# stephane-caron/pink

Hardware: AMD Instinct MI355X
Metric: ik_qp_solves_per_s (higher is better)
Workload: dtype f64

## Files before the change

### emu/wave_emu.h

```cpp
#pragma once

#include <ucontext.h>

#include <cmath>
#include <cstdio>
#include <cstdlib>
#include <cstring>

#define __device__
#define __host__
#define __global__ inline
#define __forceinline__ inline
#define __launch_bounds__(x)
#define PINKHIP_OCCUPANCY_ATTR(NV)
#define PINKHIP_OCCUPANCY_PACKED(NV, DENSE)
#define PINKHIP_OCCUPANCY_SWEEP(NT)
#define PINKHIP_OCCUPANCY_SWEEP3(NV, MD, W)
#define PINKHIP_OCCUPANCY_SWEEPX(NV, MD)
#define PINKHIP_OCCUPANCY_ROLLOUT(NV)
#define PINKHIP_OCCUPANCY_FK
#define PINKHIP_OCCUPANCY_SMALL_STACK

#include "../pink_amd/csrc/fast_sincos.h"

struct EmuDim3 {
  unsigned x = 0, y = 0, z = 0;
};
static EmuDim3 blockIdx, threadIdx;

inline unsigned long long atomicMin(unsigned long long *p, unsigned long long v) {
  const unsigned long long old = *p;
  if (v < old) *p = v;
  return old;
}

namespace pinkhip {

constexpr int kWave = 64;

struct Emu {
  int cur = 0;
  long long block = 0;
  ucontext_t main_ctx;
  ucontext_t ctx[kWave];
  bool done[kWave];
  int live = 0;
  double slot_d[kWave];
  int slot_i[kWave];
  long long arrivals[kWave];
  int tag[kWave];
  alignas(16) double lds[20480];
  char *stacks = nullptr;
};

inline Emu &emu() {
  static Emu e;
  return e;
}

inline int lane_id() { return emu().cur; }
inline long long block_id() { return emu().block; }
inline double *shared_base() { return emu().lds; }

inline void emu_rendezvous(int tag) {
  Emu &e = emu();
  const int me = e.cur;
  e.arrivals[me]++;
  e.tag[me] = tag;
  int nxt = me;
  do {
    nxt = (nxt + 1) % kWave;
  } while (e.done[nxt] && nxt != me);
  if (nxt != me) {
    e.cur = nxt;
    swapcontext(&e.ctx[me], &e.ctx[nxt]);
  }
  for (int l = 0; l < kWave; ++l) {
    if (e.done[l]) continue;
    if (e.arrivals[l] != e.arrivals[me] && e.arrivals[l] != e.arrivals[me] + 1 &&
        e.arrivals[l] + 1 != e.arrivals[me]) {
      std::fprintf(stderr, "wave emulator: divergence at lane %d vs %d (tag %d vs %d)\n", me, l,
                   e.tag[me], e.tag[l]);
      std::abort();
    }
    if (e.arrivals[l] == e.arrivals[me] && e.tag[l] != e.tag[me]) {
      std::fprintf(stderr, "wave emulator: lanes %d and %d at different primitives (%d vs %d)\n", me,
                   l, e.tag[me], e.tag[l]);
      std::abort();
    }
  }
}

inline void wave_sync() { emu_rendezvous(1); }
inline void sched_fence() {}
inline void pin16(const double (&)[8], const double (&)[8]) {}
inline void pin8(const double (&)[4], const double (&)[4]) {}
template <typename T>
inline void pin(T &) {}
inline void opaque(double &) {}
inline int opaque_uniform(int x) { return x; }
template <class Args>
inline const Args *kernarg_reload(const Args &a) {
  return &a;
}

inline double bcast(double v, int src) {
  Emu &e = emu();
  e.slot_d[e.cur] = v;
  emu_rendezvous(2);
  if (src < 0 || src >= kWave) {
    std::fprintf(stderr, "wave emulator: bcast from lane %d\n", src);
    std::abort();
  }
  const double r = e.slot_d[src];
  emu_rendezvous(3);
  return r;
}

inline int bcast_i(int v, int src) {
  Emu &e = emu();
  e.slot_i[e.cur] = v;
  emu_rendezvous(4);
  if (src < 0 || src >= kWave) std::abort();
  const int r = e.slot_i[src];
  emu_rendezvous(5);
  return r;
}

inline double emu_exchange(double v, int partner_of_me, int tag) {
  Emu &e = emu();
  e.slot_d[e.cur] = v;
  emu_rendezvous(tag);
  const double o = e.slot_d[partner_of_me];
  emu_rendezvous(tag + 1);
  return o;
}

template <class Op>
inline double emu_reduce(double v, double ident, Op op, int tag) {
  const int l = emu().cur;
  v = op(v, emu_exchange(v, l ^ 1, tag));
  v = op(v, emu_exchange(v, l ^ 2, tag));
  v = op(v, emu_exchange(v, (l & ~7) | (7 - (l & 7)), tag));
  v = op(v, emu_exchange(v, (l & ~15) | (15 - (l & 15)), tag));
  const int row = l >> 4;
  double t = emu_exchange(v, (row == 1 || row == 3) ? (row - 1) * 16 + 15 : l, tag);
  v = op(v, (row == 1 || row == 3) ? t : ident);
  t = emu_exchange(v, 31, tag);
  v = op(v, (row >= 2) ? t : ident);
  return bcast(v, 63);
}
inline double wave_sum(double v) {
  return emu_reduce(v, 0.0, [](double a, double b) { return a + b; }, 6);
}
inline double wave_min(double v) {
  return emu_reduce(v, INFINITY, [](double a, double b) { return std::fmin(a, b); }, 8);
}

inline double key_pack(double v, int payload) {
  long long b;
  std::memcpy(&b, &v, 8);
  b = (b & ~0xFFLL) | (long long)(payload & 0xFF);
  std::memcpy(&v, &b, 8);
  return v;
}
inline int key_payload(double k) {
  long long b;
  std::memcpy(&b, &k, 8);
  return (int)(b & 0xFF);
}
inline double fast_rcp(double x) { return 1.0 / x; }
inline double fast_rsqrt(double x) { return 1.0 / std::sqrt(x); }
inline double fast_rcp1(double x) { return 1.0 / x; }
inline double max_raw(double a, double b) { return a > b ? a : b; }
inline double min_raw(double a, double b) { return a < b ? a : b; }
inline int wave_uniform(int v) { return v; }
inline double approx_rcp(double x) { return 1.0 / x; }
inline float approx_rcpf(float x) { return 1.0f / x; }
inline double fast_rsqrt1(double x) { return 1.0 / std::sqrt(x); }

inline bool wave_any(bool p) {
  Emu &e = emu();
  e.slot_i[e.cur] = p ? 1 : 0;
  emu_rendezvous(14);
  bool r = false;
  for (int l = 0; l < kWave; ++l) r = r || e.slot_i[l];
  emu_rendezvous(15);
  return r;
}
inline bool lanes_on(bool) { return true; }
inline unsigned long long wave_ballot(bool p) {
  Emu &e = emu();
  e.slot_i[e.cur] = p ? 1 : 0;
  emu_rendezvous(42);
  unsigned long long r = 0;
  for (int l = 0; l < kWave; ++l)
    if (e.slot_i[l]) r |= 1ull << l;
  emu_rendezvous(43);
  return r;
}
inline bool lane_pred(unsigned long long mask) { return ((mask >> emu().cur) & 1ull) != 0; }
template <int W>
constexpr unsigned long long mask_lane(int J) {
  unsigned long long m = 0;
  for (int g = 0; g < 64 / W; ++g) m |= 1ull << (g * W + J);
  return m;
}
template <int W>
constexpr unsigned long long mask_lanes_below(int J) {
  const unsigned long long low = (J >= 64) ? ~0ull : ((1ull << J) - 1ull);
  unsigned long long m = 0;
  for (int g = 0; g < 64 / W; ++g) m |= low << (g * W);
  return m;
}
template <int W>
constexpr unsigned long long mask_groups(unsigned bits) {
  constexpr unsigned long long all = (W >= 64) ? ~0ull : ((1ull << (W & 63)) - 1ull);
  unsigned long long m = 0;
  for (int g = 0; g < 64 / W; ++g) m |= ((bits >> g) & 1u) ? (all << (g * W)) : 0ull;
  return m;
}
template <int W>
constexpr unsigned long long mask_groups_of_lane(unsigned long long m, int K) {
  unsigned bits = 0;
  for (int g = 0; g < 64 / W; ++g) bits |= static_cast<unsigned>((m >> (g * W + K)) & 1ull) << g;
  return mask_groups<W>(bits);
}
template <int W>
inline int group_first_lane(bool p) {
  Emu &e = emu();
  e.slot_i[e.cur] = p ? 1 : 0;
  emu_rendezvous(40);
  int r = W;
  const int base = e.cur & ~(W - 1);
  for (int l = W - 1; l >= 0; --l)
    if (e.slot_i[base + l]) r = l;
  emu_rendezvous(41);
  return r;
}
inline double lane_shfl(double v, int src_lane) {
  if (src_lane < 0 || src_lane >= kWave) {
    std::fprintf(stderr, "wave emulator: lane_shfl from lane %d\n", src_lane);
    std::abort();
  }
  return emu_exchange(v, src_lane, 16);
}
inline int lane_shfl_i(int v, int src_lane) {
  Emu &e = emu();
  if (src_lane < 0 || src_lane >= kWave) std::abort();
  e.slot_i[e.cur] = v;
  emu_rendezvous(18);
  const int r = e.slot_i[src_lane];
// ... 229 lines not shown
```

### pink_amd/csrc/ik_stack_rows.h

```cpp
#pragma once

#include "ik_common.h"

namespace pinkhip {

struct HbmTerms {
  static constexpr bool kOnTheFly = false;
  double lb = 0.0, ub = 0.0, x = 0.0;
  int status = 0;
  __device__ __forceinline__ void frame_rows(int, double (&)[6]) const {}
  __device__ __forceinline__ double error(int) const { return 0.0; }
  __device__ __forceinline__ double diag_error(int) const { return 0.0; }
  __device__ __forceinline__ double dense_col(int) const { return 0.0; }
  __device__ __forceinline__ double dense_h(int) const { return 0.0; }
};

struct NoMid {
  __device__ __forceinline__ void operator()() const {}
};
template <int NX>
struct StackFront {
  double m[NX > 0 ? NX : 1] = {};
  double hxx[NX > 0 ? NX * (NX + 1) / 2 : 1] = {};
  double cx[NX > 0 ? NX : 1] = {};
};
struct WaveSplit {
  long long first = 0;
  unsigned rel = 0;
};
#ifndef PINKHIP_WAVE_SPLIT
#define PINKHIP_WAVE_SPLIT(Src) (!Src::kOnTheFly)
#endif
template <int NV, int W, int RCMAX, class Src, int DEPTH = 1, int NX = 0, bool DIAG = false, int NM, class Mid = NoMid>
__device__ __forceinline__ void stack_rows_bcast(const KernelArgs &a, long long b, Src *terms, bool in, int li,
                                                 double (&M)[NM], double &ci, double &mu_l, Mid mid = Mid(), StackFront<NX> *front = nullptr,
                                                 double *hdiag = nullptr, WaveSplit ws = WaveSplit()) {
  static_assert(NX >= 0 && NX <= 2 && (NX == 0 || !Src::kOnTheFly), "at most two front columns, from HBM");
  static_assert(NM >= NV && W >= 16, "row-group kernels only");
  using BcT = Bcast<W>;
  const int nv = a.nv, Kd = a.Kd, K = a.K;
  constexpr bool SPLIT = DIAG && PINKHIP_WAVE_SPLIT(Src);
  const double *Jb = a.J + (SPLIT ? ws.first : b) * (long long)Kd * nv;
  const double *eb = a.e + (SPLIT ? ws.first : b) * (long long)K;
  const double *costb = a.cost_batched ? a.cost + (SPLIT ? ws.first : b) * (long long)K : a.cost;
  const unsigned voJ = SPLIT ? ws.rel * static_cast<unsigned>(Kd * nv) + li : 0u;
  const unsigned voE = SPLIT ? ws.rel * static_cast<unsigned>(K) + li : 0u;
  const unsigned voC = (SPLIT && a.cost_batched) ? voE : static_cast<unsigned>(li);
  constexpr int RC = Src::kOnTheFly ? 6 : (RCMAX < 8 ? RCMAX : 8);
  constexpr int NB = Src::kOnTheFly ? 2 : DEPTH + 1;
  static_assert(RC <= 16, "weight rows are broadcast from the first row of 16 lanes");
  struct Chunk {
    double r[RC];
    double pw, pe, pg, pl;
    double px[NX > 0 ? NX : 1];
  };
  Chunk buf[NB];
  auto request = [&](Chunk &dst, int r0) {
    const int rc = (Kd - r0 < RC) ? Kd - r0 : RC;
    if constexpr (Src::kOnTheFly) {
      double six[6];
      terms->frame_rows(r0 / 6, six);
#pragma unroll
      for (int kk = 0; kk < RC; ++kk) dst.r[kk] = (in && kk < rc) ? six[kk] : 0.0;
    } else {
#pragma unroll
      for (int kk = 0; kk < RC; ++kk) {
        if constexpr (SPLIT) dst.r[kk] = (in && kk < rc) ? (Jb + (long long)(r0 + kk) * nv)[voJ] : 0.0;
        else dst.r[kk] = (in && kk < rc) ? Jb[(long long)(r0 + kk) * nv + li] : 0.0;
      }
    }
    dst.pw = dst.pe = dst.pg = dst.pl = 0.0;
    if constexpr (NX > 0) {
#pragma unroll
      for (int x = 0; x < NX; ++x) {
        if constexpr (SPLIT) dst.px[x] = (li < rc) ? (Jb + ((long long)r0 * nv - NX + x))[voJ - li + static_cast<unsigned>(li * nv)] : 0.0;
        else dst.px[x] = (li < rc) ? Jb[(long long)(r0 + li) * nv - NX + x] : 0.0;
      }
    }
    if (li < rc) {
      const int k = r0 + li;
      if constexpr (SPLIT) {
        dst.pw = (costb + r0)[voC];
        if constexpr (Src::kOnTheFly) dst.pe = terms->error(k);
        else dst.pe = (eb + r0)[voE];
        dst.pg = (a.row_gain + r0)[static_cast<unsigned>(li)];
        dst.pl = (a.row_lm + r0)[static_cast<unsigned>(li)];
      } else {
        dst.pw = costb[k];
        if constexpr (Src::kOnTheFly) dst.pe = terms->error(k);
        else dst.pe = eb[k];
        dst.pg = a.row_gain[k];
        dst.pl = a.row_lm[k];
      }
    }
  };
  if (Kd > 0) {
#pragma unroll
    for (int d = 0; d < NB - 1; ++d)
      if (d * RC < Kd) request(buf[d], d * RC);
  }
  mid();
  for (int r0 = 0; r0 < Kd; r0 += RC) {
    const int rc = (Kd - r0 < RC) ? Kd - r0 : RC;
    if (r0 + (NB - 1) * RC < Kd) request(buf[NB - 1], r0 + (NB - 1) * RC);
    const Chunk &cur = buf[0];
    const double wa = (li < rc) ? cur.pw * cur.pw : 0.0;
    const double gw = (li < rc) ? cur.pg * wa * cur.pe : 0.0;
    if (li < rc) mu_l += cur.pl * (cur.pg * cur.pg) * wa * cur.pe * cur.pe;
    const BcT wab = bcast_prepare<W>(wa), gwb = bcast_prepare<W>(gw);
    BcT pxb[NX > 0 ? NX : 1];
    if constexpr (NX > 0) {
      front->hxx[0] = fma(wa * cur.px[0], cur.px[0], front->hxx[0]);
      front->cx[0] = fma(gw, cur.px[0], front->cx[0]);
      if constexpr (NX == 2) {
        front->hxx[1] = fma(wa * cur.px[0], cur.px[1], front->hxx[1]);
        front->hxx[2] = fma(wa * cur.px[1], cur.px[1], front->hxx[2]);
        front->cx[1] = fma(gw, cur.px[1], front->cx[1]);
      }
#pragma unroll
      for (int x = 0; x < NX; ++x) pxb[x] = bcast_prepare<W>(cur.px[x]);
    }
    static_for<0, RC>([&](auto Kc) {
      constexpr int kk = decltype(Kc)::value;
      if (kk < rc) {
        const double aa = fma_bcast<W, kk>(0.0, wab, cur.r[kk]);
        ci = fma_bcast<W, kk>(ci, gwb, cur.r[kk]);
        if constexpr (DIAG) *hdiag = fma(cur.r[kk], aa, *hdiag);
        const BcT rowb = bcast_prepare<W>(cur.r[kk]);
        static_for<0, NV>([&](auto Jc) {
          constexpr int j = decltype(Jc)::value;
          M[j] = fma_bcast<W, j>(M[j], rowb, aa);
        });
        if constexpr (NX > 0) {
#pragma unroll
          for (int x = 0; x < NX; ++x) front->m[x] = fma_bcast<W, kk>(front->m[x], pxb[x], aa);
        }
      }
    });
#pragma unroll
    for (int d = 0; d + 1 < NB; ++d) buf[d] = buf[d + 1];
  }
}

template <class Src>
__device__ __forceinline__ double stack_diag_tasks(const KernelArgs &a, long long b, Src *terms, int li, double &ci,
                                                   double &mu_l) {
  const double *eb = a.e + b * (long long)a.K;
  const double *costb = a.cost_batched ? a.cost + b * (long long)a.K : a.cost;
  double dadd = 0.0;
  for (int t = 0; t < a.n_dtasks; ++t) {
    const int off = li - a.dtask_col0[t];
    if (off >= 0 && off < a.dtask_k[t]) {
      const int r = a.dtask_row0[t] + off;
      const double w = costb[r], gn = a.row_gain[r], l = a.row_lm[r];
      double ev;
      if constexpr (Src::kOnTheFly) ev = terms->diag_error(r);
      else ev = eb[r];
      const double wa = w * w;
      dadd += wa;
      ci += gn * wa * ev;
      mu_l += l * (gn * gn) * wa * ev * ev;
    }
  }
  return dadd;
}

template <class Src>
__device__ __forceinline__ double stack_diag_tasks(const KernelArgs &a, WaveSplit ws, Src *terms, int li, double &ci,
                                                   double &mu_l) {
  const double *eb = a.e + ws.first * (long long)a.K;
  const double *costb = a.cost_batched ? a.cost + ws.first * (long long)a.K : a.cost;
  const unsigned vo = ws.rel * static_cast<unsigned>(a.K);
  const unsigned voc = a.cost_batched ? vo : 0u;
  double dadd = 0.0;
  for (int t = 0; t < a.n_dtasks; ++t) {
    const int off = li - a.dtask_col0[t];
    if (off >= 0 && off < a.dtask_k[t]) {
      const int r = a.dtask_row0[t] + off;
      const double w = costb[voc + static_cast<unsigned>(r)], gn = a.row_gain[r], l = a.row_lm[r];
      double ev;
      if constexpr (Src::kOnTheFly) ev = terms->diag_error(r);
      else ev = eb[vo + static_cast<unsigned>(r)];
      const double wa = w * w;
      dadd += wa;
      ci += gn * wa * ev;
      mu_l += l * (gn * gn) * wa * ev * ev;
    }
  }
  return dadd;
}

}
```

### pink_amd/csrc/ik_sweep.h

```cpp
#pragma once

#include "ik_common.h"
#include "ik_kernels_packed.h"
#include "ik_stack_rows.h"

#ifdef PINKHIP_SECTION_CLOCK
#ifndef PINKHIP_TICK
static __device__ unsigned long long pinkhip_clock[16];
#define PINKHIP_TICK(k)                                                        \
  do {                                                                         \
    if (clock_on) {                                                            \
      const unsigned long long now_ = __builtin_readcyclecounter();            \
      if (lane == 0) atomicAdd(&pinkhip_clock[k], now_ - clock_prev);          \
      clock_prev = __builtin_readcyclecounter();                               \
    }                                                                          \
  } while (0)
#endif
#else
#ifndef PINKHIP_TICK
#define PINKHIP_TICK(k)
#endif
#endif

#ifndef PINKHIP_SWEEP_COLUMN_CHAINS
#define PINKHIP_SWEEP_COLUMN_CHAINS(NT) 2
#endif

#ifndef PINKHIP_SWEEP_CERT_TOL
#define PINKHIP_SWEEP_CERT_TOL 1e-12
#endif
#ifndef PINKHIP_STACK_DEPTH
#define PINKHIP_STACK_DEPTH 1
#endif
#ifndef PINKHIP_STACK_DEPTH_WIDE
#define PINKHIP_STACK_DEPTH_WIDE 2
#endif
#ifndef PINKHIP_SWEEP_INDEXED_COLUMN
#define PINKHIP_SWEEP_INDEXED_COLUMN 1
#endif
#ifndef PINKHIP_SWEEP_ROUTE_COND
#define PINKHIP_SWEEP_ROUTE_COND 1e8
#endif
#ifndef PINKHIP_SWEEP_PPM
#define PINKHIP_SWEEP_PPM 1
#endif
#ifndef PINKHIP_SWEEP_PPM_CRASH
#define PINKHIP_SWEEP_PPM_CRASH 1
#endif
#ifndef PINKHIP_ROLLOUT_PPM_DENSE
#define PINKHIP_ROLLOUT_PPM_DENSE 0
#endif
#ifndef PINKHIP_ROLLOUT_PPM_VIRTUAL
#define PINKHIP_ROLLOUT_PPM_VIRTUAL 0
#endif
#ifndef PINKHIP_SWEEP_PPM_DENSE
#define PINKHIP_SWEEP_PPM_DENSE 1
#endif
#ifdef PINKHIP_SWEEP_DEBUG_WHY
#define PINKHIP_WHY(k) why = (k) + 10 * status_before
#else
#define PINKHIP_WHY(k)
#endif
#ifndef PINKHIP_SWEEP_PPM_MIN_CURV
#define PINKHIP_SWEEP_PPM_MIN_CURV 1e-5
#endif
#ifndef PINKHIP_SWEEP_PPM_MURTY_AFTER
#define PINKHIP_SWEEP_PPM_MURTY_AFTER(nv) (4 * (nv) + 20)
#endif

#ifndef PINKHIP_SWEEP_DIAG_REGISTER
#define PINKHIP_SWEEP_DIAG_REGISTER(Src) (!Src::kOnTheFly)
#endif
#ifndef PINKHIP_SWEEP_LATE_ADDRESSES
#define PINKHIP_SWEEP_LATE_ADDRESSES(Src) (!Src::kOnTheFly)
#endif
#ifndef PINKHIP_SWEEP_LANE_MASKS
#define PINKHIP_SWEEP_LANE_MASKS(Src) (!Src::kOnTheFly)
#endif
#ifndef PINKHIP_SWEEP_SPLIT_CLOSING
#define PINKHIP_SWEEP_SPLIT_CLOSING(Src) (!Src::kOnTheFly)
#endif

namespace pinkhip {

template <int NV, int MD, int W>
struct SweepLds {
  static __host__ __device__ constexpr int tri(int i) { return i * (i + 1) / 2; }
  static constexpr int oC = (NV * (NV + 1) / 2 + 1) & ~1;
  static constexpr int GP = W + 2;
  static constexpr int oG = oC + W;
  static constexpr int oR = oG + MD * GP;
  static constexpr int stride = oR + W;
};

template <int NVT, int MD, int W, class Src = HbmTerms, bool WARM = false>
__device__ __forceinline__ int ik_sweep_instance(const KernelArgs &a, long long block, Src *terms = nullptr) {
  constexpr int NE = NVT > W ? NVT - W : 0;
  constexpr int NV = NVT - NE;
  static_assert(NE == 0 || (NE <= 2 && MD == 0 && !Src::kOnTheFly), "front coordinates are eliminated in the box-only stack + solve kernel");
  constexpr int NT = NV + MD;
  static_assert((W == 16 || W == 32 || W == 64) && NT <= W && NV % 2 == 0 && MD >= 0, "group of whole rows of 16 lanes");
  constexpr bool DENSE = MD > 0;
  constexpr bool DREG = PINKHIP_SWEEP_DIAG_REGISTER(Src);
  constexpr bool LM = PINKHIP_SWEEP_LANE_MASKS(Src);
  constexpr bool PPM = !DENSE && PINKHIP_SWEEP_PPM;
  constexpr bool PPMD = DENSE && PINKHIP_SWEEP_PPM && PINKHIP_SWEEP_PPM_DENSE && (!Src::kOnTheFly || PINKHIP_ROLLOUT_PPM_DENSE);
  constexpr bool PPX = PPM || PPMD;
  constexpr bool LMP = LM && PPM;
  constexpr bool SPLIT = LMP && PINKHIP_SWEEP_SPLIT_CLOSING(Src);
  static_assert(!WARM || PPM, "a warm start is a start of the principal pivoting of the box-only instantiations");
  constexpr int G = kWave / W;
  constexpr double INF = INFINITY;
  constexpr double BIG = 1e300;
  using BcT = Bcast<W>;

  const int lane = lane_id();
  const int g = lane / W, li = lane & (W - 1);
  const int nvs = a.nv;
  const int nv = nvs - NE;
  const int md = DENSE ? a.md : 0, n_eq = DENSE ? a.n_eq : 0;
#ifdef PINKHIP_SECTION_CLOCK
  const bool clock_on = (block & 63) == 0;
  unsigned long long clock_prev = __builtin_readcyclecounter();
#endif
  long long b = block * G + g;
  const bool valid = b < a.B;
  if (!valid) b = a.B - 1;
  WaveSplit ws;
  ws.first = (block * G < a.B - 1) ? block * G : a.B - 1;
  ws.rel = static_cast<unsigned>(b - ws.first);
  const unsigned vo = ws.rel * static_cast<unsigned>(nvs) + li;

  const bool in = li < nv;
  const int dr = li - NV;
  const bool dlane = DENSE && dr >= 0 && dr < md;

  double T[NT];
#pragma unroll
  for (int j = 0; j < NT; ++j) T[j] = 0.0;
  double ci = 0.0, mu_l = 0.0, dadd = 0.0;
  double ci_d = 0.0, mu_d = 0.0, lbv = -INF, ubv = INF, hv = 0.0, ginv = 1.0;
  double front_dadd[NE > 0 ? NE : 1] = {}, front_c[NE > 0 ? NE : 1] = {};
  bool front_free = true;
  auto others = [&]() {
    if (in) {
      if constexpr (!Src::kOnTheFly) {
        lbv = (a.lb + (ws.first * (long long)nvs + NE))[vo];
        ubv = (a.ub + (ws.first * (long long)nvs + NE))[vo];
      }
      if constexpr (PINKHIP_WAVE_SPLIT(Src)) dadd = stack_diag_tasks<Src>(a, ws, terms, NE + li, ci_d, mu_d);
      else dadd = stack_diag_tasks<Src>(a, b, terms, NE + li, ci_d, mu_d);
      if constexpr (PINKHIP_WAVE_SPLIT(Src)) {
        if (a.c_extra) ci_d += (a.c_extra + (ws.first * (long long)nvs + NE))[vo];
      } else {
        if (a.c_extra) ci_d += a.c_extra[b * (long long)nvs + NE + li];
      }
    }
    if constexpr (NE > 0) {
#pragma unroll
      for (int x = 0; x < NE; ++x) {
        double mu_x = 0.0;
        front_dadd[x] = stack_diag_tasks<Src>(a, b, terms, x, front_c[x], mu_x);
        if (a.c_extra) front_c[x] += a.c_extra[b * (long long)nvs + x];
        if (li == x) mu_d += mu_x;
        front_free = front_free && a.lb[b * (long long)nvs + x] == -INF && a.ub[b * (long long)nvs + x] == INF;
      }
    }
    if constexpr (DENSE && !Src::kOnTheFly) {
      if (md > 0) {
        const double *Gb = a.Gd + b * (long long)md * nv;
        static_for<0, MD>([&](auto Dc) {
          constexpr int d = decltype(Dc)::value;
          T[NV + d] = (in && d < md) ? Gb[(long long)d * nv + li] : 0.0;
        });
        if (dlane) hv = a.hd[b * (long long)md + dr];
      }
    }
  };
  StackFront<NE> front;
  double hii = 0.0;
  if constexpr (NE > 0) {
    KernelArgs af = a;
    af.J = a.J + NE;
    stack_rows_bcast<NV, W, 8, Src, PINKHIP_STACK_DEPTH, NE, DREG>(af, b, terms, in, li, T, ci, mu_l, others, &front, &hii, ws);
  } else {
    stack_rows_bcast<NV, W, 8, Src, (NT > 34 ? PINKHIP_STACK_DEPTH_WIDE : PINKHIP_STACK_DEPTH), 0, DREG>(a, b, terms, in, li, T, ci, mu_l, others, nullptr, &hii, ws);
  }
  ci += ci_d;
  mu_l += mu_d;
  double diag = a.damping + group_sum<W>(mu_l);

  if constexpr (DENSE) {
    if (md > 0) {
      const double *Gb = Src::kOnTheFly ? nullptr : a.Gd + b * (long long)md * nv;
      if constexpr (Src::kOnTheFly) {
        static_for<0, MD>([&](auto Dc) {
          constexpr int d = decltype(Dc)::value;
          T[NV + d] = (in && d < md) ? terms->dense_col(d) : 0.0;
        });
      }
      if constexpr (Src::kOnTheFly) {
        static_for<0, MD>([&](auto Dc) {
          constexpr int d = decltype(Dc)::value;
          if (d < md) {
            const BcT gb = bcast_prepare<W>(T[NV + d]);
            static_for<0, NV>([&](auto Jc) {
              constexpr int j = decltype(Jc)::value;
              const double v = value_bcast<W, j>(gb);
              if (dr == d) T[j] = v;
            });
          }
        });
      }
      if (dlane) {
        double n2 = 0.0;
        if constexpr (!Src::kOnTheFly) {
          const double *gr = Gb + (long long)dr * nv;
#pragma unroll
          for (int j = 0; j < NV; ++j) T[j] = (j < nv) ? gr[j] : 0.0;
        } else {
          hv = terms->dense_h(dr);
        }
#pragma unroll
        for (int j = 0; j < NV; ++j) n2 += T[j] * T[j];
        ginv = (n2 > 0.0) ? 1.0 / sqrt(n2) : 1.0;
      }
      for (int t = 0; t < a.n_barriers; ++t) {
        const double r = a.barrier_safe_gain[t];
        if (r > 1e-6) {
          const int r0 = a.barrier_rows[t], r1 = a.barrier_rows[t + 1];
          double s = 0.0;
          static_for<0, MD>([&](auto Dc) {
            constexpr int d = decltype(Dc)::value;
            if (in && d >= r0 && d < r1) s += T[NV + d] * T[NV + d];
          });
          s = group_sum<W>(s);
          diag += r / (s * a.dt * a.dt);
        }
      }
    }
  }
  const double diag_u = diag;
  diag += dadd;
  if constexpr (DREG) {
    const double dd = in ? diag : 1.0;
    static_for<0, NV>([&](auto Jc) {
      constexpr int j = decltype(Jc)::value;
      T[j] = add_in_lane<W, j>(T[j], dd);
    });
    hii += dd;
  } else {
    hii = 1.0;
#pragma unroll
    for (int j = 0; j < NV; ++j)
      if (j == li) {
        T[j] += in ? diag : 1.0;
        hii = T[j];
      }
  }
  using SL = SweepLds<NV, MD, W>;
  double *sm = shared_base() + (long long)g * (a.lds_pitch ? a.lds_pitch : SL::stride);
  bool front_bad = false;
  if constexpr (NE > 0) {
    double h00 = group_sum<W>(front.hxx[0]) + diag_u + front_dadd[0];
    double c0 = group_sum<W>(front.cx[0]) + front_c[0];
    double h01 = 0.0, h11 = 1.0, c1 = 0.0;
    if constexpr (NE == 2) {
      h01 = group_sum<W>(front.hxx[1]);
      h11 = group_sum<W>(front.hxx[2]) + diag_u + front_dadd[1];
      c1 = group_sum<W>(front.cx[1]) + front_c[1];
    }
    const double m0 = in ? front.m[0] : 0.0;
    double m1 = (NE == 2 && in) ? front.m[NE - 1] : 0.0;
    front_bad = !(h00 > 0.0);
    const double r0 = fast_rcp(h00);
    {
      const BcT hb = bcast_prepare<W>(m0);
      const double f = -m0 * r0;
      static_for<0, NV>([&](auto Jc) {
        constexpr int j = decltype(Jc)::value;
        T[j] = fma_bcast<W, j>(T[j], hb, f);
      });
      ci = fma(f, c0, ci);
      hii = fma(f, m0, hii);
      if constexpr (NE == 2) {
        m1 = fma(f, h01, m1);
        h11 = fma(-h01 * r0, h01, h11);
        c1 = fma(-h01 * r0, c0, c1);
      }
    }
    double r1 = 0.0;
    if constexpr (NE == 2) {
      front_bad = front_bad || !(h11 > 0.0);
      r1 = fast_rcp(h11);
      const BcT hb = bcast_prepare<W>(m1);
      const double f = -m1 * r1;
      static_for<0, NV>([&](auto Jc) {
        constexpr int j = decltype(Jc)::value;
        T[j] = fma_bcast<W, j>(T[j], hb, f);
      });
      ci = fma(f, c1, ci);
      hii = fma(f, m1, hii);
    }
    wave_sync();
    sm[SL::stride + li] = m0;
    sm[SL::stride + W + li] = m1;
    if (li == 0) {
      double *fs = sm + SL::stride + 2 * W;
      fs[0] = c0, fs[1] = r0, fs[2] = h01, fs[3] = c1, fs[4] = r1;
    }
  }
  wave_sync();
  if (li < NV) {
#pragma unroll
    for (int j = 0; j < NV; ++j)
      if (j <= li) sm[SL::tri(li) + j] = T[j];
  }
  sm[SL::oC + li] = ci;
  if constexpr (DENSE) {
    static_for<0, MD>([&](auto Dc) {
      constexpr int d = decltype(Dc)::value;
      sm[SL::oG + d * SL::GP + li] = (li < NV) ? T[NV + d] : 0.0;
    });
  }
  PINKHIP_TICK(0);

  int status = STATUS_OPTIMAL;
  int why = 0, status_before = 0;
  if constexpr (NE > 0) {
    if (!front_free) status = STATUS_ROUTED;
    else if (front_bad) status = STATUS_NOT_PD;
  }
  double pmin = INF;
  int state = 0;
  if constexpr (Src::kOnTheFly) {
    lbv = in ? terms->lb : -INF;
    ubv = in ? terms->ub : INF;
  }
  constexpr bool GUESS = (PPX && PINKHIP_SWEEP_PPM_CRASH && !Src::kOnTheFly) || WARM;
// ... 1015 lines not shown
```

### pink_amd/csrc/wave.h

```cpp
#pragma once
#include <hip/hip_runtime.h>

#include "fast_sincos.h"

#ifndef PINKHIP_WAVES_SMALL
#define PINKHIP_WAVES_SMALL 4
#endif
#ifndef PINKHIP_WAVES_LARGE
#define PINKHIP_WAVES_LARGE 2
#endif
#ifndef PINKHIP_WAVES_PACKED_SMALL
#define PINKHIP_WAVES_PACKED_SMALL 4
#endif
#ifndef PINKHIP_WAVES_PACKED_LARGE
#define PINKHIP_WAVES_PACKED_LARGE 3
#endif
#define PINKHIP_OCCUPANCY_ATTR(NV) \
  __attribute__((amdgpu_waves_per_eu((NV) <= 32 ? PINKHIP_WAVES_SMALL : PINKHIP_WAVES_LARGE, \
                                     (NV) <= 32 ? PINKHIP_WAVES_SMALL : PINKHIP_WAVES_LARGE)))
#define PINKHIP_PACKED_WAVES(NV) \
  ((NV) <= 16 ? PINKHIP_WAVES_PACKED_SMALL : (NV) <= 34 ? PINKHIP_WAVES_PACKED_LARGE : PINKHIP_WAVES_LARGE)
#define PINKHIP_PACKED_WAVES2(NV, DENSE)                         \
  (((NV) == 40 && !(DENSE)) ? PINKHIP_WAVES_PACKED_LARGE         \
   : ((NV) == 24 && !(DENSE)) ? PINKHIP_WAVES_PACKED_LARGE + 1   \
                              : PINKHIP_PACKED_WAVES(NV))
#define PINKHIP_OCCUPANCY_PACKED(NV, DENSE) \
  __attribute__((amdgpu_waves_per_eu(PINKHIP_PACKED_WAVES2(NV, DENSE), PINKHIP_PACKED_WAVES2(NV, DENSE))))

#ifndef PINKHIP_SWEEP_WAVES
#ifndef PINKHIP_SWEEP_WAVES_MID
#define PINKHIP_SWEEP_WAVES_MID 3
#endif
#define PINKHIP_SWEEP_WAVES(NT) ((NT) <= 16 ? 4 : (NT) <= 34 ? PINKHIP_SWEEP_WAVES_MID : 2)
#endif
#define PINKHIP_OCCUPANCY_SWEEP(NT) __attribute__((amdgpu_waves_per_eu(PINKHIP_SWEEP_WAVES(NT), PINKHIP_SWEEP_WAVES(NT))))
#ifndef PINKHIP_SWEEP_ELIM_WAVES
#define PINKHIP_SWEEP_ELIM_WAVES 2
#endif
#define PINKHIP_OCCUPANCY_SWEEP3(NV, MD, W)                                                                             \
  __attribute__((amdgpu_waves_per_eu(((NV) > (W) ? PINKHIP_SWEEP_ELIM_WAVES : PINKHIP_SWEEP_WAVES((NV) + (MD))),     \
                                     ((NV) > (W) ? PINKHIP_SWEEP_ELIM_WAVES : PINKHIP_SWEEP_WAVES((NV) + (MD))))))
#ifndef PINKHIP_SWEEPX_WAVES
#define PINKHIP_SWEEPX_WAVES(NV, MD) ((NV) + 2 * (MD) <= 16 ? 4 : (NV) + 2 * (MD) <= 34 ? 3 : 2)
#endif
#define PINKHIP_OCCUPANCY_SWEEPX(NV, MD) \
  __attribute__((amdgpu_waves_per_eu(PINKHIP_SWEEPX_WAVES(NV, MD), PINKHIP_SWEEPX_WAVES(NV, MD))))

#ifndef PINKHIP_ROLLOUT_WAVES_SMALL
#define PINKHIP_ROLLOUT_WAVES_SMALL 3
#endif
#define PINKHIP_ROLLOUT_WAVES(NV) ((NV) <= 16 ? PINKHIP_ROLLOUT_WAVES_SMALL : PINKHIP_PACKED_WAVES(NV))
#define PINKHIP_OCCUPANCY_ROLLOUT(NV) \
  __attribute__((amdgpu_waves_per_eu(PINKHIP_ROLLOUT_WAVES(NV), PINKHIP_ROLLOUT_WAVES(NV))))

#ifndef PINKHIP_FK_WAVES
#define PINKHIP_FK_WAVES 3
#endif
#define PINKHIP_OCCUPANCY_FK __attribute__((amdgpu_waves_per_eu(PINKHIP_FK_WAVES, PINKHIP_FK_WAVES)))

#ifndef PINKHIP_SMALL_STACK_WAVES
#define PINKHIP_SMALL_STACK_WAVES 3
#endif
#define PINKHIP_OCCUPANCY_SMALL_STACK \
  __attribute__((amdgpu_waves_per_eu(PINKHIP_SMALL_STACK_WAVES, PINKHIP_SMALL_STACK_WAVES)))

namespace pinkhip {

constexpr int kWave = 64;

__device__ __forceinline__ int lane_id() { return static_cast<int>(threadIdx.x); }
__device__ __forceinline__ long long block_id() { return static_cast<long long>(blockIdx.x); }
__device__ __forceinline__ void wave_sync() {
#ifdef PINKHIP_HEAVY_SYNC
  __syncthreads();
#else
  __builtin_amdgcn_fence(__ATOMIC_RELEASE, "wavefront");
  __builtin_amdgcn_wave_barrier();
  __builtin_amdgcn_fence(__ATOMIC_ACQUIRE, "wavefront");
#endif
}

__device__ __forceinline__ double *shared_base() {
  extern __shared__ __attribute__((aligned(16))) double pinkhip_lds[];
  return pinkhip_lds;
}

template <class Args>
__device__ __forceinline__ const Args *kernarg_reload(const Args &a) {
#if defined(__HIP_DEVICE_COMPILE__)
  const Args *p = reinterpret_cast<const Args *>(__builtin_amdgcn_kernarg_segment_ptr());
  asm volatile("" : "+s"(p));
  return p;
#else
  return &a;
#endif
}

__device__ __forceinline__ void sched_fence() {
  asm volatile("" ::: "memory");
  __builtin_amdgcn_sched_barrier(0);
}

template <typename T>
__device__ __forceinline__ void pin(T &x) {
  asm volatile("" : "+v"(x) : : "memory");
}

__device__ __forceinline__ void opaque(double &x) { asm volatile("" : "+v"(x)); }

__device__ __forceinline__ int opaque_uniform(int x) {
  asm volatile("" : "+s"(x));
  return x;
}

__device__ __forceinline__ void pin16(const double (&a)[8], const double (&b)[8]) {
  asm volatile(""
               :
               : "v"(a[0]), "v"(a[1]), "v"(a[2]), "v"(a[3]), "v"(a[4]), "v"(a[5]), "v"(a[6]), "v"(a[7]), "v"(b[0]),
                 "v"(b[1]), "v"(b[2]), "v"(b[3]), "v"(b[4]), "v"(b[5]), "v"(b[6]), "v"(b[7])
               : "memory");
}

__device__ __forceinline__ void pin8(const double (&a)[4], const double (&b)[4]) {
  asm volatile("" : : "v"(a[0]), "v"(a[1]), "v"(a[2]), "v"(a[3]), "v"(b[0]), "v"(b[1]), "v"(b[2]), "v"(b[3]) : "memory");
}

__device__ __forceinline__ double bcast(double v, int src) {
  int lo = __double2loint(v), hi = __double2hiint(v);
  lo = __builtin_amdgcn_readlane(lo, src);
  hi = __builtin_amdgcn_readlane(hi, src);
  return __hiloint2double(hi, lo);
}
__device__ __forceinline__ int bcast_i(int v, int src) { return __builtin_amdgcn_readlane(v, src); }

template <int CTRL>
__device__ __forceinline__ double dpp_mov(double v) {
  int lo = __double2loint(v), hi = __double2hiint(v);
  lo = __builtin_amdgcn_update_dpp(0, lo, CTRL, 0xF, 0xF, true);
  hi = __builtin_amdgcn_update_dpp(0, hi, CTRL, 0xF, 0xF, true);
  return __hiloint2double(hi, lo);
}
__device__ __forceinline__ double min_raw(double a, double b) {
  double r;
  asm("v_min_f64 %0, %1, %2" : "=v"(r) : "v"(a), "v"(b));
  return r;
}
__device__ __forceinline__ double max_raw(double a, double b) {
  double r;
  asm("v_max_f64 %0, %1, %2" : "=v"(r) : "v"(a), "v"(b));
  return r;
}
__device__ __forceinline__ float min_raw32(float a, float b) {
  float r;
  asm("v_min_f32 %0, %1, %2" : "=v"(r) : "v"(a), "v"(b));
  return r;
}
constexpr int kDppXor1 = 0xB1;
constexpr int kDppXor2 = 0x4E;
constexpr int kDppHalfMirror = 0x141;
constexpr int kDppMirror = 0x140;

__device__ __forceinline__ double dpp_row_bcast15(double v, double ident) {
  int lo = __double2loint(v), hi = __double2hiint(v);
  lo = __builtin_amdgcn_update_dpp(__double2loint(ident), lo, 0x142, 0xA, 0xF, false);
  hi = __builtin_amdgcn_update_dpp(__double2hiint(ident), hi, 0x142, 0xA, 0xF, false);
  return __hiloint2double(hi, lo);
}
__device__ __forceinline__ double dpp_row_bcast31(double v, double ident) {
  int lo = __double2loint(v), hi = __double2hiint(v);
  lo = __builtin_amdgcn_update_dpp(__double2loint(ident), lo, 0x143, 0xC, 0xF, false);
  hi = __builtin_amdgcn_update_dpp(__double2hiint(ident), hi, 0x143, 0xC, 0xF, false);
  return __hiloint2double(hi, lo);
}

__device__ __forceinline__ double wave_sum(double v) {
  v += dpp_mov<kDppXor1>(v);
  v += dpp_mov<kDppXor2>(v);
  v += dpp_mov<kDppHalfMirror>(v);
  v += dpp_mov<kDppMirror>(v);
  v += dpp_row_bcast15(v, 0.0);
  v += dpp_row_bcast31(v, 0.0);
  return bcast(v, 63);
}

__device__ __forceinline__ double wave_min(double v) {
  v = fmin(v, dpp_mov<kDppXor1>(v));
  v = fmin(v, dpp_mov<kDppXor2>(v));
  v = fmin(v, dpp_mov<kDppHalfMirror>(v));
  v = fmin(v, dpp_mov<kDppMirror>(v));
  v = fmin(v, dpp_row_bcast15(v, INFINITY));
  v = fmin(v, dpp_row_bcast31(v, INFINITY));
  return bcast(v, 63);
}

__device__ __forceinline__ double key_pack(double v, int payload) {
  const long long b = (__double_as_longlong(v) & ~0xFFLL) | (long long)(payload & 0xFF);
  return __longlong_as_double(b);
}
__device__ __forceinline__ int key_payload(double k) { return (int)(__double_as_longlong(k) & 0xFF); }

__device__ __forceinline__ double fast_rcp(double x) {
  double r = __builtin_amdgcn_rcp(x);
  double e = fma(-x, r, 1.0);
  r = fma(r, e, r);
  e = fma(-x, r, 1.0);
  return fma(r, e, r);
}
__device__ __forceinline__ double fast_rsqrt(double x) {
  double y = __builtin_amdgcn_rsq(x);
  double e = fma(-(x * y), y, 1.0);
  y = fma(0.5 * y, e, y);
  e = fma(-(x * y), y, 1.0);
  return fma(0.5 * y, e, y);
}

__device__ __forceinline__ double fast_rcp1(double x) {
  double r = __builtin_amdgcn_rcp(x);
  const double e = fma(-x, r, 1.0);
  return fma(r, e, r);
}
__device__ __forceinline__ double fast_rsqrt1(double x) {
  double y = __builtin_amdgcn_rsq(x);
  const double e = fma(-(x * y), y, 1.0);
  return fma(0.5 * y, e, y);
}

__device__ __forceinline__ double approx_rcp(double x) { return __builtin_amdgcn_rcp(x); }
__device__ __forceinline__ float approx_rcpf(float x) { return __builtin_amdgcn_rcpf(x); }

__device__ __forceinline__ bool wave_any(bool p) { return __any(p ? 1 : 0) != 0; }
#ifdef PINKHIP_LANES_ON_SELECT
__device__ __forceinline__ bool lanes_on(bool) { return true; }
#else
__device__ __forceinline__ bool lanes_on(bool p) { return p; }
#endif
__device__ __forceinline__ unsigned long long wave_ballot(bool p) { return __builtin_amdgcn_ballot_w64(p); }
__device__ __forceinline__ int wave_uniform(int v) { return __builtin_amdgcn_readfirstlane(v); }

__device__ __forceinline__ bool lane_pred(unsigned long long mask) {
#if defined(__HIP_DEVICE_COMPILE__)
  return __builtin_amdgcn_inverse_ballot_w64(mask);
#else
  return (mask >> (threadIdx.x & 63)) & 1;
#endif
}
template <int W>
__host__ __device__ constexpr unsigned long long mask_lane(int J) {
  unsigned long long m = 0;
  for (int g = 0; g < 64 / W; ++g) m |= 1ull << (g * W + J);
  return m;
}
template <int W>
__host__ __device__ constexpr unsigned long long mask_lanes_below(int J) {
  const unsigned long long low = (J >= 64) ? ~0ull : ((1ull << J) - 1ull);
  unsigned long long m = 0;
  for (int g = 0; g < 64 / W; ++g) m |= low << (g * W);
  return m;
}
template <int W>
__host__ __device__ constexpr unsigned long long mask_groups(unsigned bits) {
  constexpr unsigned long long all = (W >= 64) ? ~0ull : ((1ull << (W & 63)) - 1ull);
// ... 250 lines not shown
```

Before: 197.8 million.

## Rotate stack-row prefetch buffers by role and skip all-zero weighted rows

In the wave-split diagonal path, the stacked-row accumulation loop now unrolls over NB chunk slots and rotates buffer roles instead of copying buffers down each iteration. A new `forget` asm marks dead slots so their registers can be released. The path also ballots across the wave to find rows whose weight and gain are zero and whose values are finite, then skips their rank-1 updates. This trades extra ballot and branch overhead, plus larger unrolled code that may raise register pressure, for fewer register moves and fewer FMAs. The rotation is disabled for NV=30, MD=8, W=64.

```diff
diff --git a/emu/wave_emu.h b/emu/wave_emu.h
--- a/emu/wave_emu.h
+++ b/emu/wave_emu.h
@@ -98,6 +98,7 @@
 template <typename T>
 inline void pin(T &) {}
 inline void opaque(double &) {}
+inline void forget(double &) {}
 inline int opaque_uniform(int x) { return x; }
 template <class Args>
 inline const Args *kernarg_reload(const Args &a) {
diff --git a/pink_amd/csrc/ik_stack_rows.h b/pink_amd/csrc/ik_stack_rows.h
--- a/pink_amd/csrc/ik_stack_rows.h
+++ b/pink_amd/csrc/ik_stack_rows.h
@@ -31,7 +31,13 @@
 #ifndef PINKHIP_WAVE_SPLIT
 #define PINKHIP_WAVE_SPLIT(Src) (!Src::kOnTheFly)
 #endif
-template <int NV, int W, int RCMAX, class Src, int DEPTH = 1, int NX = 0, bool DIAG = false, int NM, class Mid = NoMid>
+#ifndef PINKHIP_STACK_ROLE_BUFFERS
+#define PINKHIP_STACK_ROLE_BUFFERS(Src) PINKHIP_WAVE_SPLIT(Src)
+#endif
+#ifndef PINKHIP_STACK_SKIP_ZERO_ROWS
+#define PINKHIP_STACK_SKIP_ZERO_ROWS(Src) PINKHIP_WAVE_SPLIT(Src)
+#endif
+template <int NV, int W, int RCMAX, class Src, int DEPTH = 1, int NX = 0, bool DIAG = false, bool ROLE_OK = true, int NM, class Mid = NoMid>
 __device__ __forceinline__ void stack_rows_bcast(const KernelArgs &a, long long b, Src *terms, bool in, int li,
                                                  double (&M)[NM], double &ci, double &mu_l, Mid mid = Mid(), StackFront<NX> *front = nullptr,
                                                  double *hdiag = nullptr, WaveSplit ws = WaveSplit()) {
@@ -40,6 +46,8 @@
   using BcT = Bcast<W>;
   const int nv = a.nv, Kd = a.Kd, K = a.K;
   constexpr bool SPLIT = DIAG && PINKHIP_WAVE_SPLIT(Src);
+  constexpr bool ROLES = SPLIT && ROLE_OK && PINKHIP_STACK_ROLE_BUFFERS(Src);
+  constexpr bool ZSKIP = SPLIT && PINKHIP_STACK_SKIP_ZERO_ROWS(Src);
   const double *Jb = a.J + (SPLIT ? ws.first : b) * (long long)Kd * nv;
   const double *eb = a.e + (SPLIT ? ws.first : b) * (long long)K;
   const double *costb = a.cost_batched ? a.cost + (SPLIT ? ws.first : b) * (long long)K : a.cost;
@@ -94,51 +102,142 @@
       }
     }
   };
+  auto forget_chunk = [&](Chunk &dst) {
+#pragma unroll
+    for (int kk = 0; kk < RC; ++kk) forget(dst.r[kk]);
+    forget(dst.pw), forget(dst.pe), forget(dst.pg), forget(dst.pl);
+#pragma unroll
+    for (int x = 0; x < NX; ++x) forget(dst.px[x]);
+  };
   if (Kd > 0) {
 #pragma unroll
     for (int d = 0; d < NB - 1; ++d)
       if (d * RC < Kd) request(buf[d], d * RC);
   }
   mid();
-  for (int r0 = 0; r0 < Kd; r0 += RC) {
-    const int rc = (Kd - r0 < RC) ? Kd - r0 : RC;
-    if (r0 + (NB - 1) * RC < Kd) request(buf[NB - 1], r0 + (NB - 1) * RC);
-    const Chunk &cur = buf[0];
-    const double wa = (li < rc) ? cur.pw * cur.pw : 0.0;
-    const double gw = (li < rc) ? cur.pg * wa * cur.pe : 0.0;
-    if (li < rc) mu_l += cur.pl * (cur.pg * cur.pg) * wa * cur.pe * cur.pe;
-    const BcT wab = bcast_prepare<W>(wa), gwb = bcast_prepare<W>(gw);
-    BcT pxb[NX > 0 ? NX : 1];
-    if constexpr (NX > 0) {
-      front->hxx[0] = fma(wa * cur.px[0], cur.px[0], front->hxx[0]);
-      front->cx[0] = fma(gw, cur.px[0], front->cx[0]);
-      if constexpr (NX == 2) {
-        front->hxx[1] = fma(wa * cur.px[0], cur.px[1], front->hxx[1]);
-        front->hxx[2] = fma(wa * cur.px[1], cur.px[1], front->hxx[2]);
-        front->cx[1] = fma(gw, cur.px[1], front->cx[1]);
-      }
-#pragma unroll
-      for (int x = 0; x < NX; ++x) pxb[x] = bcast_prepare<W>(cur.px[x]);
-    }
-    static_for<0, RC>([&](auto Kc) {
-      constexpr int kk = decltype(Kc)::value;
-      if (kk < rc) {
-        const double aa = fma_bcast<W, kk>(0.0, wab, cur.r[kk]);
-        ci = fma_bcast<W, kk>(ci, gwb, cur.r[kk]);
-        if constexpr (DIAG) *hdiag = fma(cur.r[kk], aa, *hdiag);
-        const BcT rowb = bcast_prepare<W>(cur.r[kk]);
-        static_for<0, NV>([&](auto Jc) {
-          constexpr int j = decltype(Jc)::value;
-          M[j] = fma_bcast<W, j>(M[j], rowb, aa);
+  if constexpr (!ROLES && !ZSKIP) {
+    for (int r0 = 0; r0 < Kd; r0 += RC) {
+      const int rc = (Kd - r0 < RC) ? Kd - r0 : RC;
+      if (r0 + (NB - 1) * RC < Kd) request(buf[NB - 1], r0 + (NB - 1) * RC);
+      const Chunk &cur = buf[0];
+      const double wa = (li < rc) ? cur.pw * cur.pw : 0.0;
+      const double gw = (li < rc) ? cur.pg * wa * cur.pe : 0.0;
+      if (li < rc) mu_l += cur.pl * (cur.pg * cur.pg) * wa * cur.pe * cur.pe;
+      const BcT wab = bcast_prepare<W>(wa), gwb = bcast_prepare<W>(gw);
+      BcT pxb[NX > 0 ? NX : 1];
+      if constexpr (NX > 0) {
+        front->hxx[0] = fma(wa * cur.px[0], cur.px[0], front->hxx[0]);
+        front->cx[0] = fma(gw, cur.px[0], front->cx[0]);
+        if constexpr (NX == 2) {
+          front->hxx[1] = fma(wa * cur.px[0], cur.px[1], front->hxx[1]);
+          front->hxx[2] = fma(wa * cur.px[1], cur.px[1], front->hxx[2]);
+          front->cx[1] = fma(gw, cur.px[1], front->cx[1]);
+        }
+#pragma unroll
+        for (int x = 0; x < NX; ++x) pxb[x] = bcast_prepare<W>(cur.px[x]);
+      }
+      static_for<0, RC>([&](auto Kc) {
+        constexpr int kk = decltype(Kc)::value;
+        if (kk < rc) {
+          const double aa = fma_bcast<W, kk>(0.0, wab, cur.r[kk]);
+          ci = fma_bcast<W, kk>(ci, gwb, cur.r[kk]);
+          if constexpr (DIAG) *hdiag = fma(cur.r[kk], aa, *hdiag);
+          const BcT rowb = bcast_prepare<W>(cur.r[kk]);
+          static_for<0, NV>([&](auto Jc) {
+            constexpr int j = decltype(Jc)::value;
+            M[j] = fma_bcast<W, j>(M[j], rowb, aa);
+          });
+          if constexpr (NX > 0) {
+#pragma unroll
+            for (int x = 0; x < NX; ++x) front->m[x] = fma_bcast<W, kk>(front->m[x], pxb[x], aa);
+          }
+        }
+      });
+#pragma unroll
+      for (int d = 0; d + 1 < NB; ++d) buf[d] = buf[d + 1];
+    }
+  } else {
+    auto accumulate = [&](const Chunk &cur, int r0) {
+      const int rc = (Kd - r0 < RC) ? Kd - r0 : RC;
+      const double wa = (li < rc) ? cur.pw * cur.pw : 0.0;
+      const double gw = (li < rc) ? cur.pg * wa * cur.pe : 0.0;
+      if (li < rc) mu_l += cur.pl * (cur.pg * cur.pg) * wa * cur.pe * cur.pe;
+      unsigned live = rc >= RC ? (1u << RC) - 1u : (1u << rc) - 1u;
+      if constexpr (ZSKIP) {
+        unsigned long long cand = wave_ballot(wa == 0.0 && gw == 0.0);
+#pragma unroll
+        for (int g = 1; g < kWave / W; ++g) cand &= cand >> (W & 63);
+        unsigned c = static_cast<unsigned>(cand) & live;
+        if (opaque_uniform(static_cast<int>(c)) != 0) {
+          if constexpr (NX > 0) {
+            bool pf = fabs(cur.px[0]) < INFINITY;
+            if constexpr (NX == 2) pf = pf && fabs(cur.px[1]) < INFINITY;
+            unsigned long long pm = wave_ballot(pf);
+#pragma unroll
+            for (int g = 1; g < kWave / W; ++g) pm &= pm >> (W & 63);
+            c &= static_cast<unsigned>(pm);
+          }
+          static_for<0, RC>([&](auto Kc) {
+            constexpr int kk = decltype(Kc)::value;
+            if ((c >> kk) & 1u) {
+              if (wave_ballot(!(fabs(cur.r[kk]) < INFINITY)) == 0ull) live &= ~(1u << kk);
+            }
+          });
+        }
+      }
+      const BcT wab = bcast_prepare<W>(wa), gwb = bcast_prepare<W>(gw);
+      BcT pxb[NX > 0 ? NX : 1];
+      if constexpr (NX > 0) {
+        front->hxx[0] = fma(wa * cur.px[0], cur.px[0], front->hxx[0]);
+        front->cx[0] = fma(gw, cur.px[0], front->cx[0]);
+        if constexpr (NX == 2) {
+          front->hxx[1] = fma(wa * cur.px[0], cur.px[1], front->hxx[1]);
+          front->hxx[2] = fma(wa * cur.px[1], cur.px[1], front->hxx[2]);
+          front->cx[1] = fma(gw, cur.px[1], front->cx[1]);
+        }
+#pragma unroll
+        for (int x = 0; x < NX; ++x) pxb[x] = bcast_prepare<W>(cur.px[x]);
+      }
+      static_for<0, RC>([&](auto Kc) {
+        constexpr int kk = decltype(Kc)::value;
+        if (ZSKIP ? __builtin_expect(((live >> kk) & 1u) != 0u, 1) : kk < rc) {
+          const double aa = fma_bcast<W, kk>(0.0, wab, cur.r[kk]);
+          ci = fma_bcast<W, kk>(ci, gwb, cur.r[kk]);
+          if constexpr (DIAG) *hdiag = fma(cur.r[kk], aa, *hdiag);
+          const BcT rowb = bcast_prepare<W>(cur.r[kk]);
+          static_for<0, NV>([&](auto Jc) {
+            constexpr int j = decltype(Jc)::value;
+            M[j] = fma_bcast<W, j>(M[j], rowb, aa);
+          });
+          if constexpr (NX > 0) {
+#pragma unroll
+            for (int x = 0; x < NX; ++x) front->m[x] = fma_bcast<W, kk>(front->m[x], pxb[x], aa);
+          }
+        }
+      });
+    };
+    if constexpr (ROLES) {
+      for (int r0 = 0; r0 < Kd; r0 += NB * RC) {
+        static_for<0, NB>([&](auto Sc) {
+          constexpr int s = decltype(Sc)::value;
+          const int r = r0 + s * RC;
+          if (r < Kd) {
+            if (r + (NB - 1) * RC < Kd) request(buf[(s + NB - 1) % NB], r + (NB - 1) * RC);
+            else forget_chunk(buf[(s + NB - 1) % NB]);
+            accumulate(buf[s], r);
+          } else {
+            forget_chunk(buf[(s + NB - 1) % NB]);
+          }
         });
-        if constexpr (NX > 0) {
-#pragma unroll
-          for (int x = 0; x < NX; ++x) front->m[x] = fma_bcast<W, kk>(front->m[x], pxb[x], aa);
-        }
-      }
-    });
-#pragma unroll
-    for (int d = 0; d + 1 < NB; ++d) buf[d] = buf[d + 1];
+      }
+    } else {
+      for (int r0 = 0; r0 < Kd; r0 += RC) {
+        if (r0 + (NB - 1) * RC < Kd) request(buf[NB - 1], r0 + (NB - 1) * RC);
+        accumulate(buf[0], r0);
+#pragma unroll
+        for (int d = 0; d + 1 < NB; ++d) buf[d] = buf[d + 1];
+      }
+    }
   }
 }
 
diff --git a/pink_amd/csrc/ik_sweep.h b/pink_amd/csrc/ik_sweep.h
--- a/pink_amd/csrc/ik_sweep.h
+++ b/pink_amd/csrc/ik_sweep.h
@@ -34,6 +34,9 @@
 #endif
 #ifndef PINKHIP_STACK_DEPTH_WIDE
 #define PINKHIP_STACK_DEPTH_WIDE 2
+#endif
+#ifndef PINKHIP_SWEEP_STACK_ROLE_BUFFERS
+#define PINKHIP_SWEEP_STACK_ROLE_BUFFERS(NV, MD, W) (!((NV) == 30 && (MD) == 8 && (W) == 64))
 #endif
 #ifndef PINKHIP_SWEEP_INDEXED_COLUMN
 #define PINKHIP_SWEEP_INDEXED_COLUMN 1
@@ -182,9 +185,9 @@
   if constexpr (NE > 0) {
     KernelArgs af = a;
     af.J = a.J + NE;
-    stack_rows_bcast<NV, W, 8, Src, PINKHIP_STACK_DEPTH, NE, DREG>(af, b, terms, in, li, T, ci, mu_l, others, &front, &hii, ws);
+    stack_rows_bcast<NV, W, 8, Src, PINKHIP_STACK_DEPTH, NE, DREG, PINKHIP_SWEEP_STACK_ROLE_BUFFERS(NVT, MD, W)>(af, b, terms, in, li, T, ci, mu_l, others, &front, &hii, ws);
   } else {
-    stack_rows_bcast<NV, W, 8, Src, (NT > 34 ? PINKHIP_STACK_DEPTH_WIDE : PINKHIP_STACK_DEPTH), 0, DREG>(a, b, terms, in, li, T, ci, mu_l, others, nullptr, &hii, ws);
+    stack_rows_bcast<NV, W, 8, Src, (NT > 34 ? PINKHIP_STACK_DEPTH_WIDE : PINKHIP_STACK_DEPTH), 0, DREG, PINKHIP_SWEEP_STACK_ROLE_BUFFERS(NVT, MD, W)>(a, b, terms, in, li, T, ci, mu_l, others, nullptr, &hii, ws);
   }
   ci += ci_d;
   mu_l += mu_d;
diff --git a/pink_amd/csrc/wave.h b/pink_amd/csrc/wave.h
--- a/pink_amd/csrc/wave.h
+++ b/pink_amd/csrc/wave.h
@@ -107,6 +107,14 @@
 }
 
 __device__ __forceinline__ void opaque(double &x) { asm volatile("" : "+v"(x)); }
+
+__device__ __forceinline__ void forget(double &x) {
+#if defined(__HIP_DEVICE_COMPILE__)
+  asm volatile("" : "=v"(x));
+#else
+  (void)x;
+#endif
+}
 
 __device__ __forceinline__ int opaque_uniform(int x) {
   asm volatile("" : "+s"(x));
```

Result: faster. 203.4 million (median of 6 runs) (+2.8%).
